# rnpnr/ogl_beamforming

Hardware: AMD Instinct MI355X
Metric: beamformed voxels/s (and %HBM-roofline), 256-ch 3D DAS 512^3, 1/2/4/8 GPUs (higher is better)
Workload: dtype f32

## Files before the change

### ogl_beamforming_amd/csrc/das_staged.hip

```cpp
#include "das_common.h"

typedef int i32x2 __attribute__((ext_vector_type(2)));
typedef __attribute__((address_space(3))) f32x2 lds_f32x2;
typedef __attribute__((address_space(3))) f32x4 lds_f32x4;
typedef float f32x3 __attribute__((ext_vector_type(3)));
typedef __attribute__((address_space(3))) f32x3 lds_f32x3;

__device__ __forceinline__ float staged_phase_turns(float k, float index)
{
	float p = k * index;
	float e = __builtin_fmaf(k, index, -p);
	return hw_fract(p) + e;
}

__device__ __forceinline__ bool staged_tile_of(const BfSeparableArgs &q, bool global_tables, uint32_t &tu, uint32_t &tv, uint32_t &zl)
{
	const bool paired = global_tables && (q.depth_major & 4u);
	const uint32_t zchunks = (q.tiles[2] + 31u) >> 5;
	const uint32_t total = paired ? q.tiles[0] * q.tiles[1] * zchunks * 32u : q.tiles[0] * q.tiles[1] * q.tiles[2];
	const uint32_t per   = (total + 7u) / 8u;
	const uint32_t tile  = (blockIdx.x & 7u) * per + (blockIdx.x >> 3);
	if (tile >= total) return false;
	if (paired) {
		uint32_t r = tile >> 5;
		tu = r % q.tiles[0]; r /= q.tiles[0];
		zl = (r % zchunks) * 32u + (tile & 31u);
		tv = r / zchunks;
		return zl < q.tiles[2];
	}
	if (q.depth_major & 1u) {
		bf_column_walk(tile, q.tiles[0], q.tiles[2], q.walk_columns, tu, tv, zl);
	} else {
		tu = tile % q.tiles[0];
		tv = (tile / q.tiles[0]) % q.tiles[1];
		zl = tile / (q.tiles[0] * q.tiles[1]);
	}
	return true;
}

typedef __attribute__((address_space(4))) const f32x4 const_f32x4;
template <bool CW, int VS, int WS, int NL, bool UNI>
__device__ __forceinline__ void staged_body(const BfDasArgs &p, const BfSeparableArgs &q)
{
	extern __shared__ __attribute__((aligned(16))) f32x4 staged_lds[];
	constexpr uint32_t V = 1u << VS, W = 1u << WS;
	const uint32_t U = 1u << q.u_shift;
	const int C = p.channel_count, A = p.acquisition_count, S = p.sample_count;
	const int A4 = (A + 3) & ~3;
	const int chunk = (int)q.channel_chunk;
	f32x4 *stage  = staged_lds + 2;
	f32x4 *Tcs    = stage + (size_t)A4 * W + 1;
	const size_t table_rows = UNI ? 0 : (size_t)(A4 / 2) * V;
	f32x4 *R      = Tcs + table_rows;
	f32x2 *Tz     = reinterpret_cast<f32x2 *>(R + (size_t)chunk * U);
	int   *tfl    = reinterpret_cast<int *>(Tz + table_rows);
	int   *rfloor = tfl + A4;
	f32x2 *wave_range = reinterpret_cast<f32x2 *>(rfloor + ((chunk + 1) & ~1));
	const uint32_t stage_elements = (uint32_t)A4 * W;

	uint32_t tu, tv, zl;
	if (!staged_tile_of(q, UNI, tu, tv, zl)) return;
	const uint32_t z  = p.z_first + zl;

	const uint32_t u_axis = q.u_axis, v_axis = 1u - q.u_axis;
	const float denom[3] = {fmaxf(1.0f, (float)p.size[0] - 1.0f), fmaxf(1.0f, (float)p.size[1] - 1.0f),
	                        fmaxf(1.0f, (float)p.size[2] - 1.0f)};
	const float pz = (float)z / denom[2];
	const float phase_k = p.demodulation_frequency * p.inv_sampling_frequency;
	const BfTransmit t0 = p.transmits[0];
	const bool  rx_rows = (t0.flags & BF_RX_ROWS) != 0;
	[[maybe_unused]] const float rx_pitch = rx_rows ? p.pitch[1] : p.pitch[0];
	const uint32_t tid = threadIdx.x, nthreads = blockDim.x;
	if (q.depth_major & 2u) staged_violation_clear(tid);

	const unsigned char *tile_tab = UNI ? reinterpret_cast<const unsigned char *>(q.tables) + (size_t)(zl * q.tiles[1] + tv) * q.table_stride : nullptr;
	f32x2 range;
	if constexpr (UNI) {
		for (uint32_t a = tid; a < (uint32_t)A4; a += nthreads) tfl[a] = reinterpret_cast<const int *>(tile_tab)[a];
		if (tid == 0) stage[stage_elements] = f32x4{0.f, 0.f, 0.f, 0.f};
		range = *reinterpret_cast<const f32x2 *>(tile_tab + 4u * (uint32_t)A4);
	} else {
		for (uint32_t e = tid; e < (uint32_t)A4 * V; e += nthreads) {
			uint32_t a = e >> VS, iv = e & (V - 1);
			float cs_c = 0.f, cs_s = 0.f, t_idx = 0.f;
			if (a < (uint32_t)A) {
				float coord[3] = {0.f, 0.f, pz};
				coord[v_axis] = (float)(tv * V + iv) / denom[v_axis];
				float wx, wy, wz;
				m4_point(p.voxel_transform, coord[0], coord[1], coord[2], wx, wy, wz);
				const BfTransmit t = p.transmits[a];
				float dist = 0.f;
				if (!(t.flags & BF_TX_NONE)) {
					float px = (t.flags & BF_TX_ROWS) ? wy : wx;
					if (t.flags & BF_TX_PLANE) dist = px * t.sin_a + wz * t.cos_a;
					else { float ddx = px - t.focus_x, ddz = wz - t.focus_z; dist = hw_sqrt(ddx * ddx + ddz * ddz); }
				}
				t_idx = (div_speed_of_sound(dist, p) + p.time_offset) * p.sampling_frequency;
				float turns = staged_phase_turns(phase_k, t_idx);
				cs_c = hw_cos_turns(turns); cs_s = hw_sin_turns(turns);
			}
			const uint32_t pair = (a >> 1) * V + iv, half = a & 1u;
			reinterpret_cast<f32x2 *>(Tcs + pair)[half] = f32x2{cs_c, cs_s};
			reinterpret_cast<float *>(Tz + pair)[half]  = t_idx;
		}
		if (tid == 0) stage[stage_elements] = f32x4{0.f, 0.f, 0.f, 0.f};
		__syncthreads();
		{
			float lo = __builtin_inff(), hi = -__builtin_inff();
			for (uint32_t e = tid; e < (uint32_t)A * V; e += nthreads) {
				uint32_t a = e >> VS, iv = e & (V - 1);
				float v = reinterpret_cast<const float *>(Tz + (a >> 1) * V + iv)[a & 1u];
				lo = fminf(lo, v); hi = fmaxf(hi, v);
			}
			for (int off = 32; off > 0; off >>= 1) {
				lo = fminf(lo, __shfl_xor(lo, off, 64));
				hi = fmaxf(hi, __shfl_xor(hi, off, 64));
			}
			if ((tid & 63u) == 0) wave_range[tid >> 6] = f32x2{lo, hi};
		}
		__syncthreads();
		range = wave_range[0];
		for (uint32_t w = 1; w < (nthreads >> 6); w++) {
			range.x = fminf(range.x, wave_range[w].x);
			range.y = fmaxf(range.y, wave_range[w].y);
		}
	}
	{
		const float lo = range.x, hi = range.y;
		range.x = __builtin_bit_cast(float, __builtin_amdgcn_readfirstlane(__builtin_bit_cast(int, lo)));
		range.y = __builtin_bit_cast(float, __builtin_amdgcn_readfirstlane(__builtin_bit_cast(int, hi)));
	}
	for (uint32_t a = tid; !UNI && a < (uint32_t)A4; a += nthreads) {
		float *row = reinterpret_cast<float *>(Tz + (size_t)(a >> 1) * V) + (a & 1u);
		float  m   = row[0];
		#pragma unroll 4
		for (uint32_t iv = 1; iv < V; iv++) m = fminf(m, row[2 * iv]);
		float fl = __builtin_floorf(m);
		#pragma unroll 4
		for (uint32_t iv = 0; iv < V; iv++) row[2 * iv] = (row[2 * iv] - fl) - 0.5f;
		tfl[a] = (int)fl;
	}
	__syncthreads();

	auto voxel_of = [&](uint32_t thread, uint32_t &vx, uint32_t &vy, uint32_t &lane_u) {
		uint32_t lv_;
		if (u_axis == 0) { lane_u = thread & (U - 1); lv_ = thread >> q.u_shift; }
		else             { lv_ = thread & (V - 1); lane_u = thread >> VS; }
		const uint32_t gu = tu * U + lane_u, gv = tv * V + lv_;
		vx = u_axis == 0 ? gu : gv; vy = u_axis == 0 ? gv : gu;
	};
	uint32_t lu;
	bool inside;
	{
		uint32_t x0, y0;
		voxel_of(tid, x0, y0, lu);
		inside = x0 < p.size[0] && y0 < p.size[1];
	}

	f32x2 coherent   = {0.f, 0.f};
	float incoherent = 0.f;
	const f32x4   *Rl = R + lu;
	const uint32_t ulast = (uint32_t)(S - 1);
	uint32_t tcs_base = (uint32_t)(uintptr_t)(lds_f32x4 *)Tcs;
	uint32_t tz_base  = (uint32_t)(uintptr_t)(lds_f32x2 *)Tz;
	asm("" : "+s"(tcs_base), "+s"(tz_base));

	const __amdgpu_buffer_rsrc_t rf_rsrc = __builtin_amdgcn_make_buffer_rsrc(
		const_cast<void *>(p.rf), 0, (int)((uint32_t)C * (uint32_t)A * (uint32_t)S * 8u), 0x00020000);
	uint32_t stage_inv[NL];
	{
		const uint32_t windows_per_pass = nthreads >> WS;
		#pragma unroll
		for (int n = 0; n < NL; n++) {
			uint32_t a = (tid >> WS) + (uint32_t)n * windows_per_pass;
			stage_inv[n] = a < (uint32_t)A ? (a * (uint32_t)S + (uint32_t)(tfl[a] + (int)(tid & (W - 1)))) * 8u : 0x80000000u;
		}
	}
	auto stage_load = [&](int channel, int rfl, f32x2 (&regs)[NL]) {
		const uint32_t at = ((uint32_t)channel * (uint32_t)A * (uint32_t)S + (uint32_t)rfl) * 8u;
		#pragma unroll
		for (int n = 0; n < NL; n++) {
			i32x2 v = __builtin_amdgcn_raw_buffer_load_b64(rf_rsrc, (int)(stage_inv[n] + at), 0, 0);
			regs[n] = __builtin_bit_cast(f32x2, v);
		}
	};
	const float half_minus_j = 0.5f - (float)(tid & (W - 1));
	auto stage_store = [&](const f32x2 (&regs)[NL]) {
		#pragma unroll
		for (int n = 0; n < NL; n++) {
			const float sx = regs[n].x, sy = regs[n].y;
			const float nx = __builtin_bit_cast(float, __builtin_amdgcn_update_dpp(0, __builtin_bit_cast(int, sx), 0x130, 0xf, 0xf, true));
			const float ny = __builtin_bit_cast(float, __builtin_amdgcn_update_dpp(0, __builtin_bit_cast(int, sy), 0x130, 0xf, 0xf, true));
			const float dx = nx - sx, dy = ny - sy;
			const uint32_t e = tid + (uint32_t)n * nthreads;
			if (e < stage_elements) stage[e] = f32x4{__builtin_fmaf(half_minus_j, dx, sx), __builtin_fmaf(half_minus_j, dy, sy), dx, dy};
		}
	};

	typedef __attribute__((address_space(4))) const BfDasArgs const_args;
	const_args *kernel_args = (const_args *)__builtin_amdgcn_kernarg_segment_ptr();
	static_assert(__builtin_offsetof(BfDasArgs, xdc_transform) == 0, "BfDasArgs is the kernel's first argument: it sits at offset 0 of the segment");
	for (int c0 = 0; c0 < C; c0 += chunk) {
		const int cn = (C - c0) < chunk ? (C - c0) : chunk;
		__syncthreads();
		{
		const_args *ka = kernel_args;
		asm volatile("" : "+s"(ka));
		const uint32_t k_size[3] = {ka->size[0], ka->size[1], ka->size[2]};
		const float k_denom_u = fmaxf(1.0f, (float)k_size[u_axis] - 1.0f);
		const float k_pz = (float)z / fmaxf(1.0f, (float)k_size[2] - 1.0f);
		const float k_fs = ka->sampling_frequency, k_inv_c = ka->inv_speed_of_sound, k_c = ka->speed_of_sound, k_fnum = ka->f_number;
		const float k_phase = ka->demodulation_frequency * ka->inv_sampling_frequency;
		const float k_pitch = rx_rows ? ka->pitch[1] : ka->pitch[0];
		for (uint32_t e = tid; e < (uint32_t)cn * U; e += nthreads) {
			uint32_t c = (uint32_t)c0 + (e >> q.u_shift), iu = e & (U - 1);
			float coord[3] = {0.f, 0.f, k_pz};
			coord[u_axis] = (float)(tu * U + iu) / k_denom_u;
			float wx, wy, wz, xx, xy, xz;
			m4_point(ka->voxel_transform, coord[0], coord[1], coord[2], wx, wy, wz);
			m4_point(ka->xdc_transform, wx, wy, wz, xx, xy, xz);
			float lateral = rx_rows ? xy : xx;
			float dx      = lateral - (float)c * k_pitch;
			float a_arg   = __builtin_fabsf(dx * (k_fnum * hw_rcp(__builtin_fabsf(xz))));
			float r_idx = div_speed_of_sound(hw_sqrt(dx * dx + xz * xz), k_inv_c, k_c) * k_fs;
			f32x4 entry = {r_idx, 0.f, 0.f, 0.f};
			if (a_arg < 0.5f) {
				float cs    = hw_cos_turns(0.5f * a_arg);
				float apod  = cs * cs;
				float turns = staged_phase_turns(k_phase, r_idx);
				entry.y = apod * hw_cos_turns(turns);
				entry.z = apod * hw_sin_turns(turns);
				entry.w = apod;
			}
			R[e] = entry;
		}
		}
		__syncthreads();
		for (uint32_t cl = tid; cl < (uint32_t)cn; cl += nthreads) {
			const float *row = reinterpret_cast<const float *>(R + (size_t)cl * U);
			float m = row[0];
			#pragma unroll 4
			for (uint32_t iu = 1; iu < U; iu++) m = fminf(m, row[4 * iu]);
			rfloor[cl] = (int)__builtin_floorf(m);
		}
		__syncthreads();
		for (uint32_t e = tid; e < (uint32_t)cn * U; e += nthreads) {
			f32x4 entry = R[e];
			const bool lane_safe = (entry.x + range.x >= 0.f) && (entry.x + range.y < (float)(S - 1));
			entry.x -= (float)rfloor[e >> q.u_shift];
			if (!lane_safe) entry.w = -entry.w;
			R[e] = entry;
		}
		__syncthreads();

		f32x2 regs[NL];
		stage_load(c0, rfloor[0], regs);
		for (int cl = 0; cl < cn; cl++) {
			__syncthreads();
			stage_store(regs);
			__syncthreads();
			if (cl + 1 < cn) stage_load(c0 + cl + 1, rfloor[cl + 1], regs);
			if (!inside) continue;

			float r_rel, r_w;
			{
				const f32x4 r = Rl[(size_t)cl * U];
				r_rel = r.x; r_w = r.w;
			}
			if (__builtin_amdgcn_ballot_w64(r_w != 0.f) == 0) continue;
			const bool wave_safe = !(q.depth_major & 2u) && __builtin_amdgcn_ballot_w64(__builtin_signbitf(r_w)) == 0;
			f32x2 acc1 = {0.f, 0.f}, acc2 = {0.f, 0.f};
			f32x2 mag2 = {0.f, 0.f};
			auto term = [&](f32x2 cs, float pos, f32x4 tap) -> float {
				f32x2 sv = f32x2{tap.x, tap.y} + pos * f32x2{tap.z, tap.w};
				acc1 += sv.x * cs;
				acc2 += sv.y * cs;
				if constexpr (CW) return hw_sqrt(__builtin_fmaf(sv.y, sv.y, sv.x * sv.x));
				else return 0.f;
			};
			auto batches = [&](auto checked) {
				constexpr bool CHECK = decltype(checked)::value;
				uint32_t lane_id = tid;
				asm volatile("" : "+v"(lane_id));
				const uint32_t lane_v = u_axis == 0 ? lane_id >> q.u_shift : lane_id & (V - 1);
				uint32_t tcs_at = tcs_base + (lane_v << 4), tz_at = tz_base + (lane_v << 3);
				uint32_t m_bits = 0x4B000002u;
				[[maybe_unused]] bool window_left = false;
				const f32x2 rr = {r_rel, r_rel};
				const_f32x4 *uni_row = nullptr;
				if constexpr (UNI)
					uni_row = (const_f32x4 *)(uintptr_t)(tile_tab + 4u * (uint32_t)A4 + 16u +
					                                      (size_t)__builtin_amdgcn_readfirstlane((int)(tid >> 6)) * (size_t)(A4 / 4) * 48u);
				for (int a = 0; a < A4; a += 4, m_bits += 4u * W) {
					uint32_t at[4]; f32x4 tap[4];
					const float M = __builtin_bit_cast(float, m_bits);
					const f32x2 M2 = {M, M};
					f32x4 cs01, cs23; f32x2 tz01, tz23;
					if constexpr (UNI) {
						const f32x4 tz = uni_row[0];
						cs01 = uni_row[1]; cs23 = uni_row[2];
						tz01 = f32x2{tz.x, tz.y}; tz23 = f32x2{tz.z, tz.w};
						uni_row += 3;
					} else {
						cs01 = *(lds_f32x4 *)(uintptr_t)tcs_at;
						cs23 = *(lds_f32x4 *)(uintptr_t)(tcs_at + V * 16u);
						tz01 = *(lds_f32x2 *)(uintptr_t)tz_at;
						tz23 = *(lds_f32x2 *)(uintptr_t)(tz_at + V * 8u);
						tcs_at += 2u * V * 16u; tz_at += 2u * V * 8u;
					}
					const f32x2 p01 = rr + tz01, p23 = rr + tz23;
					const f32x2 y01 = p01 + M2,  y23 = p23 + M2;
					const float ys[4] = {y01.x, y01.y, y23.x, y23.y};
					#pragma unroll
					for (int k = 0; k < 4; k++) {
						const uint32_t yb = __builtin_bit_cast(uint32_t, ys[k]);
						asm("v_lshlrev_b16 %0, 4, %1" : "=v"(at[k]) : "v"(yb));
						if constexpr (CHECK) {
							uint32_t k_abs = (uint32_t)((int)(yb - m_bits) + rfloor[cl] + tfl[a + k]);
							at[k] = k_abs < ulast ? at[k] + (uint32_t)k * W * 16u : (stage_elements + 2u) * 16u;
							window_left |= __builtin_amdgcn_ballot_w64((yb - m_bits) > W - 2u) != 0ull;
						}
					}
					#pragma unroll
					for (int k = 0; k < 4; k++) tap[k] = *(lds_f32x4 *)(uintptr_t)(at[k] + (CHECK ? 0u : (uint32_t)k * W * 16u));
					const float q0 = term(f32x2{cs01.x, cs01.y}, p01.x, tap[0]);
					const float q1 = term(f32x2{cs01.z, cs01.w}, p01.y, tap[1]);
					const float q2 = term(f32x2{cs23.x, cs23.y}, p23.x, tap[2]);
					const float q3 = term(f32x2{cs23.z, cs23.w}, p23.y, tap[3]);
					if constexpr (CW) { mag2 += f32x2{q0, q1}; mag2 += f32x2{q2, q3}; }
				}
				if constexpr (CHECK) { if (window_left) staged_violation_raise(); }
			};
			if (wave_safe) batches(std::false_type{});
			else           batches(std::true_type{});
			float sum_x = acc1.x - acc2.y, sum_y = acc1.y + acc2.x;
			asm volatile("" : "+v"(sum_x), "+v"(sum_y));
			const f32x4 r = *(volatile lds_f32x4 *)(uintptr_t)((uint32_t)(uintptr_t)(lds_f32x4 *)Rl + (uint32_t)cl * U * 16u);
			coherent.x = __builtin_fmaf(sum_x, r.y, __builtin_fmaf(-sum_y, r.z, coherent.x));
			coherent.y = __builtin_fmaf(sum_x, r.z, __builtin_fmaf(sum_y, r.y, coherent.y));
			if constexpr (CW) incoherent = __builtin_fmaf(__builtin_fabsf(r.w), mag2.x + mag2.y, incoherent);
		}
	}
	if (q.depth_major & 2u) staged_violation_report(tid);
	if (!inside) return;

	uint32_t x, y, lane_u_unused, thread = tid;
	asm volatile("" : "+v"(thread));
	voxel_of(thread, x, y, lane_u_unused);
	uint64_t out_index = (uint64_t)p.size[0] * p.size[1] * zl + (uint64_t)p.size[0] * y + x;
	if constexpr (CW) coherent = coherent * (coherent / incoherent);
	reinterpret_cast<f32x2 *>(p.out)[out_index] = coherent;
}

template <bool CW, int NL>
__device__ __forceinline__ void staged_paired_body(const BfDasArgs &p, const BfSeparableArgs &q)
{
	extern __shared__ __attribute__((aligned(16))) f32x4 staged_lds[];
	constexpr uint32_t U = 32, W = 32, B = 2 * W;
	const int C = p.channel_count, A = p.acquisition_count, S = p.sample_count;
	const uint32_t A4 = ((uint32_t)A + 3u) & ~3u;
	const int chunk = (int)q.channel_chunk;
	uint32_t G0, G1;
	if (!bf_staged_paired_split(A4, q.channel_chunk, &G0, &G1)) return;
	const uint32_t ngroups = G1 ? 2u : 1u;
	f32x4 *stage  = staged_lds + 2;
	f32x4 *R      = stage + (size_t)G0 * B + 1;
	int   *tfl    = reinterpret_cast<int *>(R + (size_t)((chunk + 1) & ~1) * U);
	int   *rfloor = tfl + A4;
	uint32_t *rbase = reinterpret_cast<uint32_t *>(rfloor + ((chunk + 2) & ~1));

	uint32_t tu, tv, zl;
	if (!staged_tile_of(q, true, tu, tv, zl)) return;
	const uint32_t z = p.z_first + zl;
	const uint32_t u_axis = q.u_axis, v_axis = 1u - q.u_axis;
	const bool rx_rows = (p.transmits[0].flags & BF_RX_ROWS) != 0;
	const uint32_t tid = threadIdx.x;
	if (q.depth_major & 2u) staged_violation_clear(tid);
	auto opaque_tid = [&]() -> uint32_t { uint32_t t = tid; asm volatile("" : "+v"(t)); return t; };

	const unsigned char *tile_tab = reinterpret_cast<const unsigned char *>(q.tables) + (size_t)(zl * q.tiles[1] + tv) * q.table_stride;
	typedef __attribute__((address_space(4))) const int const_int;
	const_int *tab_floor = (const_int *)(uintptr_t)tile_tab;
	for (uint32_t a = tid; a < A4; a += 1024u) tfl[a] = reinterpret_cast<const int *>(tile_tab)[a];
	if (tid == 0) stage[(size_t)G0 * B] = f32x4{0.f, 0.f, 0.f, 0.f};
	f32x2 range = *reinterpret_cast<const f32x2 *>(tile_tab + 4u * A4);
	{
		const float lo = range.x, hi = range.y;
		range.x = __builtin_bit_cast(float, __builtin_amdgcn_readfirstlane(__builtin_bit_cast(int, lo)));
		range.y = __builtin_bit_cast(float, __builtin_amdgcn_readfirstlane(__builtin_bit_cast(int, hi)));
	}

	const uint32_t wave = (uint32_t)__builtin_amdgcn_readfirstlane((int)(tid >> 6));
	const uint32_t h = (tid >> 5) & 1u, lu = tid & 31u;
	bool inside;
	{
		const uint32_t gu = tu * U + lu, gv = tv * 32u + wave;
		inside = gu < p.size[u_axis] && gv < p.size[v_axis];
	}
	const bool wave_inside = __builtin_amdgcn_ballot_w64(inside) != 0ull;

	const __amdgpu_buffer_rsrc_t rf_rsrc = __builtin_amdgcn_make_buffer_rsrc(
		const_cast<void *>(p.rf), 0, (int)((uint32_t)C * (uint32_t)A * (uint32_t)S * 8u), 0x00020000);
	auto lane_at_of = [&](int cl) -> uint32_t { return rbase[cl] + ((opaque_tid() & 31u) << 3); };
	auto stage_load = [&](uint32_t lane_at, uint32_t g, f32x2 (&regs)[NL]) {
		const uint32_t a0 = g ? G0 : 0u, gn = g ? G1 : G0;
		int fl[NL];
		#pragma unroll
		for (int n = 0; n < NL; n++) {
			const uint32_t a = a0 + wave + (uint32_t)n * 16u;
			fl[n] = tab_floor[a < A4 ? a : A4 - 1u];
		}
		#pragma unroll
		for (int n = 0; n < NL; n++) {
			const uint32_t al = wave + (uint32_t)n * 16u, a = a0 + al;
			const bool real = al < gn && a < (uint32_t)A;
			const uint32_t off = real ? lane_at + ((a * (uint32_t)S + (uint32_t)fl[n]) * 8u) : 0x80000000u;
			i32x2 v = __builtin_amdgcn_raw_buffer_load_b64(rf_rsrc, (int)off, 0, 0);
			regs[n] = __builtin_bit_cast(f32x2, v);
		}
	};
	auto stage_store = [&](uint32_t g, const f32x2 (&regs)[NL]) {
		const uint32_t gn = g ? G1 : G0;
		const uint32_t tid = opaque_tid();
		const float half_minus_j = 0.5f - (float)(tid & 63u);
		#pragma unroll
		for (int n = 0; n < NL; n++) {
			if (wave + (uint32_t)n * 16u >= gn) break;
			const float sx = regs[n].x, sy = regs[n].y;
			const float nx = __builtin_bit_cast(float, __builtin_amdgcn_update_dpp(0, __builtin_bit_cast(int, sx), 0x130, 0xf, 0xf, true));
			const float ny = __builtin_bit_cast(float, __builtin_amdgcn_update_dpp(0, __builtin_bit_cast(int, sy), 0x130, 0xf, 0xf, true));
			const float dx = nx - sx, dy = ny - sy;
			stage[tid + (uint32_t)n * 1024u] = f32x4{__builtin_fmaf(half_minus_j, dx, sx), __builtin_fmaf(half_minus_j, dy, sy), dx, dy};
		}
	};

	f32x2 coherent   = {0.f, 0.f};
	float incoherent = 0.f;
	auto exchange = [](float x, float y) -> float {
		const auto r = __builtin_amdgcn_permlane32_swap(__builtin_bit_cast(uint32_t, x), __builtin_bit_cast(uint32_t, y), false, false);
		return __builtin_bit_cast(float, (uint32_t)r[0]) + __builtin_bit_cast(float, (uint32_t)r[1]);
	};
	const f32x4 *Rl = R + (size_t)h * U + lu;
	const uint32_t ulast = (uint32_t)(S - 1);
	const const_f32x4 *rows = (const_f32x4 *)(uintptr_t)(tile_tab + 4u * A4 + 16u) + (size_t)wave * (A4 / 2u) * 3u;

	typedef __attribute__((address_space(4))) const BfDasArgs const_args;
	const_args *kernel_args = (const_args *)__builtin_amdgcn_kernarg_segment_ptr();
	for (int c0 = 0; c0 < C; c0 += chunk) {
		const int cn = (C - c0) < chunk ? (C - c0) : chunk;
		const int cn2 = (cn + 1) & ~1;
		__syncthreads();
		{
		const_args *ka = kernel_args;
		asm volatile("" : "+s"(ka));
		const uint32_t k_size[3] = {ka->size[0], ka->size[1], ka->size[2]};
		const float k_denom_u = fmaxf(1.0f, (float)k_size[u_axis] - 1.0f);
		uint32_t k_z = z;
		asm volatile("" : "+s"(k_z));
		const float k_pz = (float)k_z / fmaxf(1.0f, (float)k_size[2] - 1.0f);
		const float k_fs = ka->sampling_frequency, k_inv_c = ka->inv_speed_of_sound, k_c = ka->speed_of_sound, k_fnum = ka->f_number;
		const float k_phase = ka->demodulation_frequency * ka->inv_sampling_frequency;
		const float k_pitch = rx_rows ? ka->pitch[1] : ka->pitch[0];
		for (uint32_t e = opaque_tid(); e < (uint32_t)cn2 * U; e += 1024u) {
			uint32_t cl = e >> 5, iu = e & (U - 1);
			f32x4 entry = {0.f, 0.f, 0.f, 0.f};
			if ((int)cl < cn) {
				uint32_t c = (uint32_t)c0 + cl;
				float coord[3] = {0.f, 0.f, k_pz};
				coord[u_axis] = (float)(tu * U + iu) / k_denom_u;
				float wx, wy, wz, xx, xy, xz;
				m4_point(ka->voxel_transform, coord[0], coord[1], coord[2], wx, wy, wz);
				m4_point(ka->xdc_transform, wx, wy, wz, xx, xy, xz);
				float lateral = rx_rows ? xy : xx;
				float dx      = lateral - (float)c * k_pitch;
				float a_arg   = __builtin_fabsf(dx * (k_fnum * hw_rcp(__builtin_fabsf(xz))));
				float r_idx = div_speed_of_sound(hw_sqrt(dx * dx + xz * xz), k_inv_c, k_c) * k_fs;
				entry.x = r_idx;
				if (a_arg < 0.5f) {
					float cs    = hw_cos_turns(0.5f * a_arg);
					float apod  = cs * cs;
					float turns = staged_phase_turns(k_phase, r_idx);
					entry.y = apod * hw_cos_turns(turns);
					entry.z = apod * hw_sin_turns(turns);
					entry.w = apod;
				}
			}
			R[e] = entry;
		}
		}
		__syncthreads();
		for (uint32_t cl = opaque_tid(); cl < (uint32_t)cn2; cl += 1024u) {
			const float *row = reinterpret_cast<const float *>(R + (size_t)cl * U);
			float m = row[0];
			#pragma unroll 4
			for (uint32_t iu = 1; iu < U; iu++) m = fminf(m, row[4 * iu]);
			const int fl = (int)__builtin_floorf(m);
			rfloor[cl] = fl;
			rbase[cl] = c0 + (int)cl < C ? ((uint32_t)(c0 + (int)cl) * (uint32_t)A * (uint32_t)S + (uint32_t)fl) * 8u : 0x80000000u;
		}
		__syncthreads();
		for (uint32_t e = opaque_tid(); e < (uint32_t)cn2 * U; e += 1024u) {
			f32x4 entry = R[e];
			const uint32_t cl = e >> 5;
			const bool lane_safe = (int)cl >= cn || ((entry.x + range.x >= 0.f) && (entry.x + range.y < (float)(S - 1)));
			entry.x = (entry.x - (float)rfloor[cl]) + (float)((cl & 1u) * W);
			if (!lane_safe) entry.w = -entry.w;
			R[e] = entry;
		}
		__syncthreads();

		f32x2 regs[NL];
		stage_load(lane_at_of((int)h), 0, regs);
		for (int k = 0; k < cn2 / 2; k++) {
			float r_rel = 0.f;
			int mode = 0;
			if (wave_inside) {
				const f32x4 r = Rl[(size_t)(2 * k) * U];
				r_rel = r.x;
				if (__builtin_amdgcn_ballot_w64(r.w != 0.f) != 0)
					mode = (!(q.depth_major & 2u) && __builtin_amdgcn_ballot_w64(__builtin_signbitf(r.w)) == 0) ? 1 : 2;
			}
			auto rounds = [&](auto mode_c) {
				constexpr int MODE = decltype(mode_c)::value;
				constexpr bool CHECK = MODE == 2;
				constexpr bool AHEAD = MODE == 1 && NL <= 3;
				f32x2 acc1a = {0.f, 0.f}, acc2a = {0.f, 0.f}, acc1b = {0.f, 0.f}, acc2b = {0.f, 0.f};
				f32x2 mag2 = {0.f, 0.f};
				for (uint32_t g = 0; g < ngroups; g++) {
					__syncthreads();
					stage_store(g, regs);
					__syncthreads();
					if (g + 1 < ngroups)     stage_load(lane_at_of(2 * k + (int)h), g + 1, regs);
					else if (2 * k + 2 < cn2) stage_load(lane_at_of(2 * k + 2 + (int)h), 0, regs);
					if constexpr (MODE != 0) {
						const uint32_t a0 = g ? G0 : 0u, gn = g ? G1 : G0;
						uint32_t m_bits = 0x4B000002u;
						[[maybe_unused]] bool window_left = false;
						[[maybe_unused]] int rfl_h = 0;
						if constexpr (CHECK) rfl_h = rfloor[2 * k + (int)h] - (int)(h * W);
						const f32x2 rr = {r_rel, r_rel};
						auto batch = [&](uint32_t a, const f32x4 tz, const f32x4 cs0, const f32x4 cs1, auto &&behind_rotates) {
							constexpr int T = 4;
							uint32_t at[T]; f32x4 tap[T]; f32x2 sv[T];
							const float M = __builtin_bit_cast(float, m_bits);
							const f32x2 M2 = {M, M};
							const f32x2 p0 = rr + f32x2{tz.x, tz.y}, p1 = rr + f32x2{tz.z, tz.w};
							const f32x2 y0 = p0 + M2, y1 = p1 + M2;
							const float ys[4] = {y0.x, y0.y, y1.x, y1.y}, ps[4] = {p0.x, p0.y, p1.x, p1.y};
							const f32x2 cs[4] = {{cs0.x, cs0.y}, {cs0.z, cs0.w}, {cs1.x, cs1.y}, {cs1.z, cs1.w}};
							#pragma unroll
							for (int t = 0; t < T; t++) {
								const uint32_t yb = __builtin_bit_cast(uint32_t, ys[t]);
								asm("v_lshlrev_b16 %0, 4, %1" : "=v"(at[t]) : "v"(yb));
								if constexpr (CHECK) {
									uint32_t lane_id = tid;
									asm volatile("" : "+v"(lane_id));
									const uint32_t rel = yb - m_bits;
									const uint32_t k_abs = (uint32_t)((int)rel + rfl_h + tfl[a0 + a + (uint32_t)(t >> 1)]);
									at[t] = k_abs < ulast ? at[t] + (uint32_t)(t >> 1) * B * 16u : (G0 * B + 2u) * 16u;
									window_left |= __builtin_amdgcn_ballot_w64(inside && rel - (lane_id & 32u) > W - 2u) != 0ull;
								}
							}
							#pragma unroll
							for (int t = 0; t < T; t++) tap[t] = *(lds_f32x4 *)(uintptr_t)(at[t] + (CHECK ? 0u : (uint32_t)(t >> 1) * B * 16u));
							[[maybe_unused]] float q[T];
							#pragma unroll
							for (int t = 0; t < T; t++) {
								sv[t] = f32x2{tap[t].x, tap[t].y} + ps[t] * f32x2{tap[t].z, tap[t].w};
								if (t & 1) { acc1b += sv[t].x * cs[t]; acc2b += sv[t].y * cs[t]; }
								else       { acc1a += sv[t].x * cs[t]; acc2a += sv[t].y * cs[t]; }
								if constexpr (CW && !AHEAD) q[t] = hw_sqrt(__builtin_fmaf(sv[t].y, sv[t].y, sv[t].x * sv[t].x));
							}
							behind_rotates();
							if constexpr (CW) {
								#pragma unroll
								for (int t = 0; AHEAD && t < T; t++) q[t] = hw_sqrt(__builtin_fmaf(sv[t].y, sv[t].y, sv[t].x * sv[t].x));
								mag2 += f32x2{q[0], q[1]}; mag2 += f32x2{q[2], q[3]};
							}
						};
						const_f32x4 *row = rows + (size_t)(a0 / 2u) * 3u;
						if constexpr (!AHEAD) {
							for (uint32_t a = 0; a < gn; a += 2, m_bits += 2u * B, row += 3) batch(a, row[0], row[1], row[2], [] {});
						} else {
							f32x4 tz = row[0], cs0 = row[1], cs1 = row[2];
							uint32_t a = 0;
							for (; a + 2u < gn; a += 2, m_bits += 2u * B)
								batch(a, tz, cs0, cs1, [&] {
									__builtin_amdgcn_sched_barrier(0);
									row += 3;
									tz = row[0]; cs0 = row[1]; cs1 = row[2];
									__builtin_amdgcn_sched_barrier(0);
								});
							batch(a, tz, cs0, cs1, [] {});
						}
						if constexpr (CHECK) { if (window_left) staged_violation_raise(); }
					}
				}
				if constexpr (MODE != 0) {
					float sa_x = acc1a.x - acc2a.y, sa_y = acc1a.y + acc2a.x;
					float sb_x = acc1b.x - acc2b.y, sb_y = acc1b.y + acc2b.x;
					asm volatile("" : "+v"(sa_x), "+v"(sa_y), "+v"(sb_x), "+v"(sb_y));
					const f32x4 r = *(volatile lds_f32x4 *)(uintptr_t)((uint32_t)(uintptr_t)(lds_f32x4 *)Rl + (uint32_t)(2 * k) * U * 16u);
					const float ca_x = __builtin_fmaf(sa_x, r.y, -sa_y * r.z), ca_y = __builtin_fmaf(sa_x, r.z, sa_y * r.y);
					const float cb_x = __builtin_fmaf(sb_x, r.y, -sb_y * r.z), cb_y = __builtin_fmaf(sb_x, r.z, sb_y * r.y);
					coherent.x += exchange(ca_x, cb_x);
					coherent.y += exchange(ca_y, cb_y);
					if constexpr (CW) incoherent += exchange(__builtin_fabsf(r.w) * mag2.x, __builtin_fabsf(r.w) * mag2.y);
				}
			};
			if (mode == 1)      rounds(std::integral_constant<int, 1>{});
			else if (mode == 2) rounds(std::integral_constant<int, 2>{});
			else                rounds(std::integral_constant<int, 0>{});
		}
	}
	if (q.depth_major & 2u) staged_violation_report(tid);
	uint32_t thread = tid;
	asm volatile("" : "+v"(thread));
	const uint32_t gu = tu * U + (thread & 31u), gv = tv * 32u + (thread >> 6) + ((thread >> 5) & 1u) * 16u;
	if (!(gu < p.size[u_axis] && gv < p.size[v_axis])) return;
	const uint32_t x = u_axis == 0 ? gu : gv, y = u_axis == 0 ? gv : gu;
	uint64_t out_index = (uint64_t)p.size[0] * p.size[1] * zl + (uint64_t)p.size[0] * y + x;
	if constexpr (CW) coherent = coherent * (coherent / incoherent);
	reinterpret_cast<f32x2 *>(p.out)[out_index] = coherent;
}

template <bool CW, int VS, int WS, int NL, bool UNI, bool PAIRED>
__global__ __launch_bounds__(1024, 8) void das_rca_staged_kernel(const BfDasArgs p, const BfSeparableArgs q)
{
	if constexpr (PAIRED) staged_paired_body<CW, NL>(p, q);
	else                  staged_body<CW, VS, WS, NL, UNI>(p, q);
}

template <bool CW, int VS, int WS, int NL, bool UNI>
static hipError_t launch_staged(const BfDasArgs *a, const BfSeparableArgs *q, hipStream_t s)
{
	uint32_t total = q->tiles[0] * q->tiles[1] * q->tiles[2];
	if (UNI && (q->depth_major & 4u)) total = q->tiles[0] * q->tiles[1] * ((q->tiles[2] + 31u) >> 5) * 32u;
	uint32_t grid  = ((total + 7u) / 8u) * 8u;
	auto kernel = das_rca_staged_kernel<CW, VS, WS, NL, UNI, false>;
	hipError_t e = hipFuncSetAttribute((const void *)kernel, hipFuncAttributeMaxDynamicSharedMemorySize, (int)q->lds_bytes);
	if (e != hipSuccess) return e;
	hipLaunchKernelGGL(kernel, dim3(grid), dim3(q->threads), q->lds_bytes, s, *a, *q);
	return hipGetLastError();
}

template <bool CW, int VS, int WS, bool UNI>
static hipError_t launch_staged_loads(const BfDasArgs *a, const BfSeparableArgs *q, hipStream_t s)
{
	const uint32_t A4 = ((uint32_t)a->acquisition_count + 3u) & ~3u;
	const uint32_t passes = ((A4 << WS) + q->threads - 1) / q->threads;
	switch (passes) {
	case 1: return launch_staged<CW, VS, WS, 1, UNI>(a, q, s);
	case 2: return launch_staged<CW, VS, WS, 2, UNI>(a, q, s);
	case 3: return launch_staged<CW, VS, WS, 3, UNI>(a, q, s);
	case 4: return launch_staged<CW, VS, WS, 4, UNI>(a, q, s);
	}
	return hipErrorInvalidValue;
}

template <bool CW, int NL>
static hipError_t launch_staged_paired(const BfDasArgs *a, const BfSeparableArgs *q, hipStream_t s)
{
	const uint32_t total = q->tiles[0] * q->tiles[1] * ((q->depth_major & 4u) ? ((q->tiles[2] + 31u) >> 5) * 32u : q->tiles[2]);
	const uint32_t grid  = ((total + 7u) / 8u) * 8u;
	auto kernel = das_rca_staged_kernel<CW, 5, 5, NL, true, true>;
	hipError_t e = hipFuncSetAttribute((const void *)kernel, hipFuncAttributeMaxDynamicSharedMemorySize, (int)q->lds_bytes);
	if (e != hipSuccess) return e;
	hipLaunchKernelGGL(kernel, dim3(grid), dim3(1024), q->lds_bytes, s, *a, *q);
	return hipGetLastError();
}

template <bool CW>
static hipError_t launch_staged_shape(const BfDasArgs *a, const BfSeparableArgs *q, hipStream_t s)
{
	if (q->uniform == 2) {
		if (q->u_shift != 5 || q->v_shift != 5 || q->window_samples != 32 || q->threads != 1024 || !q->tables ||
		    ((q->channel_chunk & 1u) && (int)q->channel_chunk < a->channel_count)) return hipErrorInvalidValue;
		const uint32_t A4 = ((uint32_t)a->acquisition_count + 3u) & ~3u;
		uint32_t G0, G1;
		if (!bf_staged_paired_split(A4, q->channel_chunk, &G0, &G1) || q->lds_bytes < bf_staged_paired_lds_bytes(G0, q->channel_chunk, A4)) return hipErrorInvalidValue;
		switch (bf_staged_paired_passes(G0)) {
		case 2: return launch_staged_paired<CW, 2>(a, q, s);
		case 3: return launch_staged_paired<CW, 3>(a, q, s);
		case 4: return launch_staged_paired<CW, 4>(a, q, s);
		}
		return hipErrorInvalidValue;
	}
	if (q->uniform) {
		if (q->u_axis != 0 || q->u_shift != 6 || q->v_shift != 4 || q->threads != 1024 || !q->tables) return hipErrorInvalidValue;
		if (q->window_samples == 32) return launch_staged_loads<CW, 4, 5, true>(a, q, s);
		if (q->window_samples == 64) return launch_staged_loads<CW, 4, 6, true>(a, q, s);
		return hipErrorInvalidValue;
	}
	switch ((q->v_shift << 4) | q->window_shift) {
	case (4 << 4) | 5: return launch_staged_loads<CW, 4, 5, false>(a, q, s);
	case (5 << 4) | 5: return launch_staged_loads<CW, 5, 5, false>(a, q, s);
	case (6 << 4) | 5: return launch_staged_loads<CW, 6, 5, false>(a, q, s);
	case (4 << 4) | 6: return launch_staged_loads<CW, 4, 6, false>(a, q, s);
	case (5 << 4) | 6: return launch_staged_loads<CW, 5, 6, false>(a, q, s);
	case (6 << 4) | 6: return launch_staged_loads<CW, 6, 6, false>(a, q, s);
	}
	return hipErrorInvalidValue;
}

extern "C" hipError_t bf_launch_das_staged(const BfDasArgs *a, const BfSeparableArgs *q, hipStream_t s)
{
	if (!a->complex_data || a->interpolation != BF_INTERP_LINEAR) return hipErrorInvalidValue;
	if ((uint64_t)a->channel_count * (uint64_t)a->acquisition_count * (uint64_t)a->sample_count * 8u >= (1ull << 31)) return hipErrorInvalidValue;
	return a->coherency_weighting ? launch_staged_shape<true>(a, q, s) : launch_staged_shape<false>(a, q, s);
}

template <int VS>
__global__ __launch_bounds__(256) void staged_tables_kernel(const BfDasArgs p, const BfSeparableArgs q)
{
	extern __shared__ __attribute__((aligned(16))) f32x4 tables_lds[];
	constexpr uint32_t V = 1u << VS;
	const int A = p.acquisition_count;
	const int A4 = (A + 3) & ~3;
	float *t  = reinterpret_cast<float *>(tables_lds);
	f32x2 *cs = reinterpret_cast<f32x2 *>(t + (size_t)A4 * V);
	f32x2 *wave_range = cs + (size_t)A4 * V;
	const uint32_t tv = blockIdx.x % q.tiles[1], zl = blockIdx.x / q.tiles[1];
	const uint32_t z  = p.z_first + zl;
	const uint32_t v_axis = 1u - q.u_axis;
	const float denom[3] = {fmaxf(1.0f, (float)p.size[0] - 1.0f), fmaxf(1.0f, (float)p.size[1] - 1.0f),
	                        fmaxf(1.0f, (float)p.size[2] - 1.0f)};
	const float pz = (float)z / denom[2];
	const float phase_k = p.demodulation_frequency * p.inv_sampling_frequency;
	const uint32_t tid = threadIdx.x, nthreads = blockDim.x;
	for (uint32_t e = tid; e < (uint32_t)A4 * V; e += nthreads) {
		uint32_t a = e >> VS, iv = e & (V - 1);
		float cs_c = 0.f, cs_s = 0.f, t_idx = 0.f;
		if (a < (uint32_t)A) {
			float coord[3] = {0.f, 0.f, pz};
			coord[v_axis] = (float)(tv * V + iv) / denom[v_axis];
			float wx, wy, wz;
			m4_point(p.voxel_transform, coord[0], coord[1], coord[2], wx, wy, wz);
			const BfTransmit t_a = p.transmits[a];
			float dist = 0.f;
			if (!(t_a.flags & BF_TX_NONE)) {
				float px = (t_a.flags & BF_TX_ROWS) ? wy : wx;
				if (t_a.flags & BF_TX_PLANE) dist = px * t_a.sin_a + wz * t_a.cos_a;
				else { float ddx = px - t_a.focus_x, ddz = wz - t_a.focus_z; dist = hw_sqrt(ddx * ddx + ddz * ddz); }
			}
			t_idx = (div_speed_of_sound(dist, p) + p.time_offset) * p.sampling_frequency;
			float turns = staged_phase_turns(phase_k, t_idx);
			cs_c = hw_cos_turns(turns); cs_s = hw_sin_turns(turns);
		}
		t[e] = t_idx; cs[e] = f32x2{cs_c, cs_s};
	}
	__syncthreads();
	{
		float lo = __builtin_inff(), hi = -__builtin_inff();
		for (uint32_t e = tid; e < (uint32_t)A * V; e += nthreads) { lo = fminf(lo, t[e]); hi = fmaxf(hi, t[e]); }
		for (int off = 32; off > 0; off >>= 1) {
			lo = fminf(lo, __shfl_xor(lo, off, 64));
			hi = fmaxf(hi, __shfl_xor(hi, off, 64));
		}
		if ((tid & 63u) == 0) wave_range[tid >> 6] = f32x2{lo, hi};
	}
	__syncthreads();
	unsigned char *tile_tab = reinterpret_cast<unsigned char *>(q.tables) + (size_t)blockIdx.x * q.table_stride;
	if (tid == 0) {
		f32x2 range = wave_range[0];
		for (uint32_t w = 1; w < (nthreads >> 6); w++) {
			range.x = fminf(range.x, wave_range[w].x);
			range.y = fmaxf(range.y, wave_range[w].y);
		}
		*reinterpret_cast<f32x4 *>(tile_tab + 4u * (uint32_t)A4) = f32x4{range.x, range.y, 0.f, 0.f};
	}
	for (uint32_t a = tid; a < (uint32_t)A4; a += nthreads) {
		float *row = t + (size_t)a * V;
		float  m   = row[0];
		for (uint32_t iv = 1; iv < V; iv++) m = fminf(m, row[iv]);
		float fl = __builtin_floorf(m);
		for (uint32_t iv = 0; iv < V; iv++) row[iv] = (row[iv] - fl) - 0.5f;
		reinterpret_cast<int *>(tile_tab)[a] = (int)fl;
	}
	__syncthreads();
	f32x4 *rows = reinterpret_cast<f32x4 *>(tile_tab + 4u * (uint32_t)A4 + 16u);
	if constexpr (VS == 5) {
		const uint32_t batches = (uint32_t)A4 / 2u;
		for (uint32_t e = tid; e < 16u * batches; e += nthreads) {
			const uint32_t w = e / batches, b = e % batches;
			const float *t2 = t + (size_t)(2u * b) * V + w;
			const f32x2 *c2 = cs + (size_t)(2u * b) * V + w;
			f32x4 *row = rows + (size_t)e * 3u;
			row[0] = f32x4{t2[0], t2[16], t2[V], t2[V + 16]};
			row[1] = f32x4{c2[0].x, c2[0].y, c2[16].x, c2[16].y};
			row[2] = f32x4{c2[V].x, c2[V].y, c2[V + 16].x, c2[V + 16].y};
		}
		return;
	}
	const uint32_t batches = (uint32_t)A4 / 4u;
	for (uint32_t e = tid; e < V * batches; e += nthreads) {
		const uint32_t iv = e / batches, b = e % batches;
		const float *t4 = t + (size_t)(4u * b) * V + iv;
		const f32x2 *c4 = cs + (size_t)(4u * b) * V + iv;
		f32x4 *row = rows + (size_t)e * 3u;
		row[0] = f32x4{t4[0], t4[V], t4[2 * V], t4[3 * V]};
		row[1] = f32x4{c4[0].x, c4[0].y, c4[V].x, c4[V].y};
		row[2] = f32x4{c4[2 * V].x, c4[2 * V].y, c4[3 * V].x, c4[3 * V].y};
	}
}

extern "C" hipError_t bf_launch_das_staged_tables(const BfDasArgs *a, const BfSeparableArgs *q, hipStream_t s)
{
	const uint32_t A4 = ((uint32_t)a->acquisition_count + 3u) & ~3u;
	if (!q->tables) return hipErrorInvalidValue;
	if (q->uniform == 1 && q->v_shift == 4) {
		if (q->table_stride < 4u * A4 + 16u + 16u * (A4 / 4u) * 48u) return hipErrorInvalidValue;
		hipLaunchKernelGGL(staged_tables_kernel<4>, dim3(q->tiles[1] * q->tiles[2]), dim3(256), A4 * 16u * 12u + 64u, s, *a, *q);
		return hipGetLastError();
	}
	if (q->uniform == 2 && q->v_shift == 5) {
		if (q->table_stride < 4u * A4 + 16u + 16u * (A4 / 2u) * 48u) return hipErrorInvalidValue;
		const uint32_t lds = A4 * 32u * 12u + 64u;
		hipError_t e = hipFuncSetAttribute((const void *)staged_tables_kernel<5>, hipFuncAttributeMaxDynamicSharedMemorySize, (int)lds);
		if (e != hipSuccess) return e;
		hipLaunchKernelGGL(staged_tables_kernel<5>, dim3(q->tiles[1] * q->tiles[2]), dim3(256), lds, s, *a, *q);
		return hipGetLastError();
	}
	return hipErrorInvalidValue;
}
```

Baseline: 182.9 million.

## Precompute staged load offsets and run same-mode channel pairs in a tight loop

Precomputes per-group RF staging offsets once as wave-uniform scalars, so the tab_floor lookups and bounds checks leave the inner stage_load. It also restructures the channel-pair loop so that consecutive pairs with the same mode stay inside one specialized loop, with the next pair's mode looked up ahead. Apertures that end mid-group are now trimmed to the real element count instead of processing padded batches. This cuts scalar and branch overhead per channel pair, at the cost of more scalar registers and extra code paths for partial batches.

```diff
diff --git a/ogl_beamforming_amd/csrc/das_staged.hip b/ogl_beamforming_amd/csrc/das_staged.hip
--- a/ogl_beamforming_amd/csrc/das_staged.hip
+++ b/ogl_beamforming_amd/csrc/das_staged.hip
@@ -402,30 +402,39 @@
 	const __amdgpu_buffer_rsrc_t rf_rsrc = __builtin_amdgcn_make_buffer_rsrc(
 		const_cast<void *>(p.rf), 0, (int)((uint32_t)C * (uint32_t)A * (uint32_t)S * 8u), 0x00020000);
 	auto lane_at_of = [&](int cl) -> uint32_t { return rbase[cl] + ((opaque_tid() & 31u) << 3); };
-	auto stage_load = [&](uint32_t lane_at, uint32_t g, f32x2 (&regs)[NL]) {
+	constexpr uint32_t STAGE_SKIP = 0x80000004u;
+	uint32_t stage_off[2][NL];
+	#pragma unroll
+	for (int g = 0; g < 2; g++) {
 		const uint32_t a0 = g ? G0 : 0u, gn = g ? G1 : G0;
-		int fl[NL];
-		#pragma unroll
-		for (int n = 0; n < NL; n++) {
-			const uint32_t a = a0 + wave + (uint32_t)n * 16u;
-			fl[n] = tab_floor[a < A4 ? a : A4 - 1u];
-		}
 		#pragma unroll
 		for (int n = 0; n < NL; n++) {
 			const uint32_t al = wave + (uint32_t)n * 16u, a = a0 + al;
-			const bool real = al < gn && a < (uint32_t)A;
-			const uint32_t off = real ? lane_at + ((a * (uint32_t)S + (uint32_t)fl[n]) * 8u) : 0x80000000u;
-			i32x2 v = __builtin_amdgcn_raw_buffer_load_b64(rf_rsrc, (int)off, 0, 0);
+			const int fl = tab_floor[a < A4 ? a : A4 - 1u];
+			uint32_t off = (a * (uint32_t)S + (uint32_t)fl) * 8u;
+			if (a >= (uint32_t)A) off = STAGE_SKIP;
+			if (al >= gn) off = STAGE_SKIP;
+			off = (uint32_t)__builtin_amdgcn_readfirstlane((int)off);
+			asm volatile("" : "+s"(off));
+			stage_off[g][n] = off;
+		}
+	}
+	auto stage_load = [&](uint32_t lane_at, uint32_t g, f32x2 (&regs)[NL]) {
+		#pragma unroll
+		for (int n = 0; n < NL; n++) {
+			const uint32_t off = g ? stage_off[1][n] : stage_off[0][n];
+			i32x2 v = __builtin_amdgcn_raw_buffer_load_b64(rf_rsrc, (int)(lane_at + off), 0, 0);
 			regs[n] = __builtin_bit_cast(f32x2, v);
 		}
 	};
 	auto stage_store = [&](uint32_t g, const f32x2 (&regs)[NL]) {
-		const uint32_t gn = g ? G1 : G0;
 		const uint32_t tid = opaque_tid();
 		const float half_minus_j = 0.5f - (float)(tid & 63u);
 		#pragma unroll
 		for (int n = 0; n < NL; n++) {
-			if (wave + (uint32_t)n * 16u >= gn) break;
+			uint32_t off = g ? stage_off[1][n] : stage_off[0][n];
+			asm volatile("" : "+s"(off));
+			if (off & 4u) break;
 			const float sx = regs[n].x, sy = regs[n].y;
 			const float nx = __builtin_bit_cast(float, __builtin_amdgcn_update_dpp(0, __builtin_bit_cast(int, sx), 0x130, 0xf, 0xf, true));
 			const float ny = __builtin_bit_cast(float, __builtin_amdgcn_update_dpp(0, __builtin_bit_cast(int, sy), 0x130, 0xf, 0xf, true));
@@ -440,7 +449,9 @@
 		const auto r = __builtin_amdgcn_permlane32_swap(__builtin_bit_cast(uint32_t, x), __builtin_bit_cast(uint32_t, y), false, false);
 		return __builtin_bit_cast(float, (uint32_t)r[0]) + __builtin_bit_cast(float, (uint32_t)r[1]);
 	};
-	const f32x4 *Rl = R + (size_t)h * U + lu;
+	uint32_t r_base = (uint32_t)(uintptr_t)(lds_f32x4 *)R;
+	asm("" : "+s"(r_base));
+	auto entry_of = [&](int k) -> uint32_t { return r_base + (uint32_t)k * (2u * U * 16u) + ((opaque_tid() & 63u) << 4); };
 	const uint32_t ulast = (uint32_t)(S - 1);
 	const const_f32x4 *rows = (const_f32x4 *)(uintptr_t)(tile_tab + 4u * A4 + 16u) + (size_t)wave * (A4 / 2u) * 3u;
 
@@ -499,49 +510,59 @@
 			rbase[cl] = c0 + (int)cl < C ? ((uint32_t)(c0 + (int)cl) * (uint32_t)A * (uint32_t)S + (uint32_t)fl) * 8u : 0x80000000u;
 		}
 		__syncthreads();
+		int k_last = S - 1;
+		asm volatile("" : "+s"(k_last));
 		for (uint32_t e = opaque_tid(); e < (uint32_t)cn2 * U; e += 1024u) {
 			f32x4 entry = R[e];
 			const uint32_t cl = e >> 5;
-			const bool lane_safe = (int)cl >= cn || ((entry.x + range.x >= 0.f) && (entry.x + range.y < (float)(S - 1)));
+			const bool lane_safe = (int)cl >= cn || ((entry.x + range.x >= 0.f) && (entry.x + range.y < (float)k_last));
 			entry.x = (entry.x - (float)rfloor[cl]) + (float)((cl & 1u) * W);
 			if (!lane_safe) entry.w = -entry.w;
 			R[e] = entry;
 		}
 		__syncthreads();
 
-		f32x2 regs[NL];
-		stage_load(lane_at_of((int)h), 0, regs);
-		for (int k = 0; k < cn2 / 2; k++) {
-			float r_rel = 0.f;
-			int mode = 0;
-			if (wave_inside) {
-				const f32x4 r = Rl[(size_t)(2 * k) * U];
-				r_rel = r.x;
-				if (__builtin_amdgcn_ballot_w64(r.w != 0.f) != 0)
-					mode = (!(q.depth_major & 2u) && __builtin_amdgcn_ballot_w64(__builtin_signbitf(r.w)) == 0) ? 1 : 2;
-			}
-			auto rounds = [&](auto mode_c) {
-				constexpr int MODE = decltype(mode_c)::value;
-				constexpr bool CHECK = MODE == 2;
-				constexpr bool AHEAD = MODE == 1 && NL <= 3;
+		const int pairs = cn2 / 2;
+		auto mode_of = [&](int k, float &r_rel) -> int {
+			if (!wave_inside) return 0;
+			const __attribute__((address_space(3))) float *r = (const __attribute__((address_space(3))) float *)(uintptr_t)entry_of(k);
+			const float r_w = r[3];
+			r_rel = r[0];
+			if (__builtin_amdgcn_ballot_w64(r_w != 0.f) == 0) return 0;
+			return (!(q.depth_major & 2u) && __builtin_amdgcn_ballot_w64(__builtin_signbitf(r_w)) == 0) ? 1 : 2;
+		};
+		float r_rel = 0.f;
+		int k = 0, mode = mode_of(0, r_rel);
+		auto run = [&](auto mode_c) {
+			constexpr int MODE = decltype(mode_c)::value;
+			constexpr bool CHECK = MODE == 2;
+			constexpr bool AHEAD = MODE == 1 && NL <= 3;
+			f32x2 regs[NL] = {};
+			stage_load(lane_at_of(2 * k + (int)h), 0, regs);
+			do {
+				float next_rel = 0.f;
+				int next_mode = -1;
+				if (k + 1 < pairs) next_mode = mode_of(k + 1, next_rel);
 				f32x2 acc1a = {0.f, 0.f}, acc2a = {0.f, 0.f}, acc1b = {0.f, 0.f}, acc2b = {0.f, 0.f};
 				f32x2 mag2 = {0.f, 0.f};
 				for (uint32_t g = 0; g < ngroups; g++) {
 					__syncthreads();
 					stage_store(g, regs);
 					__syncthreads();
-					if (g + 1 < ngroups)     stage_load(lane_at_of(2 * k + (int)h), g + 1, regs);
-					else if (2 * k + 2 < cn2) stage_load(lane_at_of(2 * k + 2 + (int)h), 0, regs);
+					if (g + 1 < ngroups) stage_load(lane_at_of(2 * k + (int)h), 1, regs);
+					else if (next_mode == MODE) stage_load(lane_at_of(2 * k + 2 + (int)h), 0, regs);
 					if constexpr (MODE != 0) {
 						const uint32_t a0 = g ? G0 : 0u, gn = g ? G1 : G0;
+						const uint32_t left = (uint32_t)A - a0, gr = left < gn ? left : gn;
 						uint32_t m_bits = 0x4B000002u;
 						[[maybe_unused]] bool window_left = false;
 						[[maybe_unused]] int rfl_h = 0;
 						if constexpr (CHECK) rfl_h = rfloor[2 * k + (int)h] - (int)(h * W);
 						const f32x2 rr = {r_rel, r_rel};
-						auto batch = [&](uint32_t a, const f32x4 tz, const f32x4 cs0, const f32x4 cs1, auto &&behind_rotates) {
-							constexpr int T = 4;
-							uint32_t at[T]; f32x4 tap[T]; f32x2 sv[T];
+						auto batch = [&](auto part_c, uint32_t a, const f32x4 tz, const f32x4 cs0, const f32x4 cs1, auto &&behind_rotates) {
+							constexpr int PART = decltype(part_c)::value;
+							constexpr int T0 = PART == 2 ? 2 : 0, T = PART == 1 ? 2 : 4;
+							uint32_t at[4]; f32x4 tap[4]; f32x2 sv[4];
 							const float M = __builtin_bit_cast(float, m_bits);
 							const f32x2 M2 = {M, M};
 							const f32x2 p0 = rr + f32x2{tz.x, tz.y}, p1 = rr + f32x2{tz.z, tz.w};
@@ -549,7 +570,7 @@
 							const float ys[4] = {y0.x, y0.y, y1.x, y1.y}, ps[4] = {p0.x, p0.y, p1.x, p1.y};
 							const f32x2 cs[4] = {{cs0.x, cs0.y}, {cs0.z, cs0.w}, {cs1.x, cs1.y}, {cs1.z, cs1.w}};
 							#pragma unroll
-							for (int t = 0; t < T; t++) {
+							for (int t = T0; t < T; t++) {
 								const uint32_t yb = __builtin_bit_cast(uint32_t, ys[t]);
 								asm("v_lshlrev_b16 %0, 4, %1" : "=v"(at[t]) : "v"(yb));
 								if constexpr (CHECK) {
@@ -562,10 +583,10 @@
 								}
 							}
 							#pragma unroll
-							for (int t = 0; t < T; t++) tap[t] = *(lds_f32x4 *)(uintptr_t)(at[t] + (CHECK ? 0u : (uint32_t)(t >> 1) * B * 16u));
-							[[maybe_unused]] float q[T];
+							for (int t = T0; t < T; t++) tap[t] = *(lds_f32x4 *)(uintptr_t)(at[t] + (CHECK ? 0u : (uint32_t)(t >> 1) * B * 16u));
+							[[maybe_unused]] float q[4] = {0.f, 0.f, 0.f, 0.f};
 							#pragma unroll
-							for (int t = 0; t < T; t++) {
+							for (int t = T0; t < T; t++) {
 								sv[t] = f32x2{tap[t].x, tap[t].y} + ps[t] * f32x2{tap[t].z, tap[t].w};
 								if (t & 1) { acc1b += sv[t].x * cs[t]; acc2b += sv[t].y * cs[t]; }
 								else       { acc1a += sv[t].x * cs[t]; acc2a += sv[t].y * cs[t]; }
@@ -574,24 +595,30 @@
 							behind_rotates();
 							if constexpr (CW) {
 								#pragma unroll
-								for (int t = 0; AHEAD && t < T; t++) q[t] = hw_sqrt(__builtin_fmaf(sv[t].y, sv[t].y, sv[t].x * sv[t].x));
-								mag2 += f32x2{q[0], q[1]}; mag2 += f32x2{q[2], q[3]};
+								for (int t = T0; AHEAD && t < T; t++) q[t] = hw_sqrt(__builtin_fmaf(sv[t].y, sv[t].y, sv[t].x * sv[t].x));
+								if constexpr (T0 == 0) mag2 += f32x2{q[0], q[1]};
+								if constexpr (T == 4)  mag2 += f32x2{q[2], q[3]};
 							}
 						};
+						constexpr std::integral_constant<int, 0> both{};
+						constexpr std::integral_constant<int, 1> first{};
+						constexpr std::integral_constant<int, 2> second{};
 						const_f32x4 *row = rows + (size_t)(a0 / 2u) * 3u;
+						uint32_t a = 0;
 						if constexpr (!AHEAD) {
-							for (uint32_t a = 0; a < gn; a += 2, m_bits += 2u * B, row += 3) batch(a, row[0], row[1], row[2], [] {});
+							for (; a + 1u < gr; a += 2, m_bits += 2u * B, row += 3) batch(both, a, row[0], row[1], row[2], [] {});
+							if (a < gr) batch(first, a, row[0], row[1], row[1], [] {});
 						} else {
 							f32x4 tz = row[0], cs0 = row[1], cs1 = row[2];
-							uint32_t a = 0;
-							for (; a + 2u < gn; a += 2, m_bits += 2u * B)
-								batch(a, tz, cs0, cs1, [&] {
+							for (; a + 2u < gr; a += 2, m_bits += 2u * B)
+								batch(both, a, tz, cs0, cs1, [&] {
 									__builtin_amdgcn_sched_barrier(0);
 									row += 3;
 									tz = row[0]; cs0 = row[1]; cs1 = row[2];
 									__builtin_amdgcn_sched_barrier(0);
 								});
-							batch(a, tz, cs0, cs1, [] {});
+							batch(first, a, tz, cs0, cs1, [] {});
+							if (a + 1u < gr) batch(second, a, tz, cs0, cs1, [] {});
 						}
 						if constexpr (CHECK) { if (window_left) staged_violation_raise(); }
 					}
@@ -600,17 +627,23 @@
 					float sa_x = acc1a.x - acc2a.y, sa_y = acc1a.y + acc2a.x;
 					float sb_x = acc1b.x - acc2b.y, sb_y = acc1b.y + acc2b.x;
 					asm volatile("" : "+v"(sa_x), "+v"(sa_y), "+v"(sb_x), "+v"(sb_y));
-					const f32x4 r = *(volatile lds_f32x4 *)(uintptr_t)((uint32_t)(uintptr_t)(lds_f32x4 *)Rl + (uint32_t)(2 * k) * U * 16u);
+					const f32x4 r = *(volatile lds_f32x4 *)(uintptr_t)entry_of(k);
 					const float ca_x = __builtin_fmaf(sa_x, r.y, -sa_y * r.z), ca_y = __builtin_fmaf(sa_x, r.z, sa_y * r.y);
 					const float cb_x = __builtin_fmaf(sb_x, r.y, -sb_y * r.z), cb_y = __builtin_fmaf(sb_x, r.z, sb_y * r.y);
 					coherent.x += exchange(ca_x, cb_x);
 					coherent.y += exchange(ca_y, cb_y);
 					if constexpr (CW) incoherent += exchange(__builtin_fabsf(r.w) * mag2.x, __builtin_fabsf(r.w) * mag2.y);
 				}
-			};
-			if (mode == 1)      rounds(std::integral_constant<int, 1>{});
-			else if (mode == 2) rounds(std::integral_constant<int, 2>{});
-			else                rounds(std::integral_constant<int, 0>{});
+				k++;
+				mode = next_mode;
+				if constexpr (NL >= 4) next_rel = mode > 0 ? *(volatile __attribute__((address_space(3))) float *)(uintptr_t)entry_of(k) : 0.f;
+				r_rel = next_rel;
+			} while (mode == MODE);
+		};
+		while (k < pairs) {
+			if (mode == 1)      run(std::integral_constant<int, 1>{});
+			else if (mode == 2) run(std::integral_constant<int, 2>{});
+			else                run(std::integral_constant<int, 0>{});
 		}
 	}
 	if (q.depth_major & 2u) staged_violation_report(tid);
```

New measurement: 186.4 million, median of 6. 1.9% higher.
